# utiasSTARS/ceres-slam

Measured on AMD Instinct MI355X. Metric: gauss_newton_iters_per_sec, higher is better.
Workload: dtype f64

## Files before the change

ceres_slam_amd/csrc/ssba_api.hip:

```cpp
#include <hip/hip_runtime.h>

#include <algorithm>
#include <chrono>
#include <cmath>
#include <cstdio>
#include <cstdlib>
#include <cstring>
#include <map>
#include <condition_variable>
#include <memory>
#include <mutex>
#include <system_error>
#include <thread>
#include <string>
#include <vector>

#include "../../include/ssba.h"
#include "ssba_pool.h"
#include <dlfcn.h>
#include <rccl/rccl.h>

#include "ssba_launch.h"
#include "ssba_layout.h"
#include "ssba_wide_layout.h"
// ... 956 lines not shown
            if (f >= 0 && (f / SBP < d.chain0 || f / SBP > d.chain1)) {
                set_error("ssba_set_partition: an observation of this rank touches a pose outside its chain of super-blocks");
                return SSBA_ERR_INVALID_ARGUMENT;
            }
        }
    }
    {
        int n = part ? d.chain1 - d.chain0 + 1 : d.Nsb, lev = 0;
        const size_t c0 = part ? (size_t)d.chain0 : 0;
        d.lev[0].n = n;
        d.lev[0].D = d.xv + d.off_D + c0 * blk;
        d.lev[0].L = d.xv + d.off_L + c0 * blk;
        d.lev[0].r = d.xv + d.off_rhs + c0 * BD;
        std::vector<int> pos(n);
        for (int i = 0; i < n; ++i) pos[i] = i;
        for (;;) {
            if (d.nb) TRY(dzero(p, &d.lev[lev].B, (size_t)d.np * n * BD * NBP));
            TRY(dzero(p, &d.lev[lev].YU, (size_t)std::max(1, n / 2) * blk));
            TRY(upload_pos(pos, &d.lev[lev].pos));
            if (part ? n <= pcr_max : n == 1) break;
            d.lev[lev].pin = (part && d.pin1 && (n % 2 == 0)) ? 1 : 0;
            const int n2 = d.lev[lev].pin ? n / 2 + 1 : (n + 1) / 2;
            std::vector<int> pos2(n2);
            for (int m = 0; m < n2; ++m) pos2[m] = (d.lev[lev].pin && m == n2 - 1) ? pos[n - 1] : pos[2 * m];
            ++lev;
            if (lev >= MAX_LEVELS) return SSBA_ERR_UNSUPPORTED;
            d.lev[lev].n = n2;
            TRY(dzero(p, &d.lev[lev].D, (size_t)n2 * blk));
            TRY(dzero(p, &d.lev[lev].L, (size_t)n2 * blk));
            TRY(dzero(p, &d.lev[lev].r, (size_t)n2 * BD));
            n = n2;
            pos.swap(pos2);
        }
        d.n_levels = lev + 1;
    }
    d.pcr.level = -1;
    auto make_pcr = [&](PcrPlan &P, int level, int n, int keep, int pin0, int pin1) -> int {
        P.level = level; P.n = n; P.steps = 0; P.keep = keep; P.pin0 = pin0; P.pin1 = pin1;
        for (int s2 = 1; s2 < n; s2 <<= 1) ++P.steps;
        const size_t slots = keep ? (size_t)std::max(P.steps, 1) * n : (size_t)n;
        TRY(dzero(p, &P.Lbuf, (size_t)n * blk)); TRY(dzero(p, &P.LbufT, (size_t)n * blk));
        TRY(dzero(p, &P.YL, slots * blk)); TRY(dzero(p, &P.YU, slots * blk));
        TRY(dzero(p, &P.yr, (size_t)n * BD));
        if (pin1) TRY(dzero(p, &P.Ubuf, (size_t)n * blk));
        if (keep) {
            TRY(dzero(p, &P.Gs, slots * blk));
            const size_t np = d.nb ? (size_t)d.np : 1;
            TRY(dzero(p, &P.Bb, np * n * BD * NBP)); TRY(dzero(p, &P.yB, np * n * BD * NBP));
        }
        return SSBA_OK;
    };
    auto make_fused = [&](PcrFused &F, size_t n, bool pins) -> int {
        for (int q = 0; q < 2; ++q) {
            TRY(dzero(p, &F.Dpp[q], n * blk)); TRY(dzero(p, &F.rpp[q], n * BD));
            TRY(dzero(p, &F.GLL[q], n * blk)); TRY(dzero(p, &F.GUU[q], n * blk));
            TRY(dzero(p, &F.GUL[q], n * blk)); TRY(dzero(p, &F.GULT[q], n * blk));
            TRY(dzero(p, &F.gL[q], n * BD)); TRY(dzero(p, &F.gU[q], n * BD));
        }
        if (pins) { TRY(dzero(p, &F.Lkeep, n * blk)); TRY(dzero(p, &F.Ukeep, n * blk)); }
        F.on = 1;
        return SSBA_OK;
    };
    {
        const char *e = getenv("SSBA_NO_PCR");
        if (part) {
            TRY(make_pcr(d.pcr, d.n_levels - 1, d.lev[d.n_levels - 1].n, 0, d.pin0, d.pin1));
            if (!d.nb) TRY(make_fused(d.pcrf, (size_t)d.pcr.n, true));
        } else if ((!d.nb || d.lev[0].n <= pcr_max) && p->world_size == 1 && !dense && !(e && e[0] == '1')) {
            int k = 0;
            while (d.lev[k].n > pcr_max) ++k;
            TRY(make_pcr(d.pcr, k, d.lev[k].n, d.nb ? 1 : 0, 0, 0));
            if (!d.nb) TRY(make_fused(d.pcrf, (size_t)d.pcr.n, false));
        }
    }
    if (part) {
        const uint64_t ns = (uint64_t)d.n_sep;
        d.soff_D = 0;
        d.soff_L = d.soff_D + ns * blk;
        d.soff_rhs = d.soff_L + ns * blk;
        d.soff_gp = d.soff_rhs + ns * BD;
        d.soff_hdiag = d.soff_gp + ns * BD;
        d.soff_scal = d.soff_hdiag + ns * BD;
        d.sepv_count = d.soff_scal + NSCAL + (uint64_t)d.world;
        TRY(dzero(p, &d.sepv, d.sepv_count));
        TRY(dzero(p, &d.xsep, (size_t)ns * BD));
        d.slev[0].n = d.n_sep;
        d.slev[0].D = d.sepv + d.soff_D;
        d.slev[0].L = d.sepv + d.soff_L;
        d.slev[0].r = d.sepv + d.soff_rhs;
        std::vector<int> pos(d.n_sep);
        for (int i = 0; i < d.n_sep; ++i) pos[i] = i;
        TRY(upload_pos(pos, &d.slev[0].pos));
        TRY(make_pcr(d.spcr, 0, d.n_sep, 0, 0, 0));
        TRY(make_fused(d.spcrf, (size_t)ns, false));
    }
    std::vector<uint32_t> dn_blk_rf_start, dn_blk_rf;
    if (!pfs.empty()) {
        std::vector<uint32_t> start(P + 1, 0);
        for (auto &f : pfs) start[f.pose + 1]++;
        for (uint32_t k = 0; k < P; ++k) start[k + 1] += start[k];
        std::vector<uint32_t> cur(start.begin(), start.end() - 1);
        const size_t F = pfs.size();
        std::vector<int> type(F);
        std::vector<double> data(F * 18), S(F * 36), hub(F);
        std::vector<uint32_t> pos(F);
        for (size_t i = 0; i < F; ++i) pos[i] = cur[pfs[i].pose]++;
        for (size_t i = 0; i < F; ++i) {
            auto &f = pfs[i];
            const uint32_t q = pos[i];
            type[q] = f.type; hub[q] = f.huber;
            memcpy(&data[18 * (size_t)q], f.data, sizeof f.data);
            if (f.type >= 2 && f.data[14] >= 0.0) data[18 * (size_t)q + 14] = (double)pos[(size_t)f.data[14]];
// ... 1466 lines not shown
```

ceres_slam_amd/csrc/ssba_bcr_mfma.hip:

```cpp
#include <hip/hip_runtime.h>
#include <math.h>
#include <stdint.h>
#include <algorithm>

#include "ssba_device.h"
#include "ssba_launch.h"
#include "ssba_types.h"

namespace ssba {

typedef double mf_d4 __attribute__((ext_vector_type(4)));

static __device__ __forceinline__ mf_d4 mf(double a, double b, mf_d4 c) { return __builtin_amdgcn_mfma_f64_16x16x4f64(a, b, c, 0, 0, 0); }
static __device__ __forceinline__ double mf_readlane(double v, int lane) {
    const int lo = __builtin_amdgcn_readlane(__double2loint(v), lane);
    const int hi = __builtin_amdgcn_readlane(__double2hiint(v), lane);
    return __hiloint2double(hi, lo);
}
static __device__ __forceinline__ double mf_rcp(double a) {
    double r = __builtin_amdgcn_rcp(a);
    return fma(fma(-a, r, 1.0), r, r);
}
static __device__ __forceinline__ double mf_rsqrt(double a) {
    double r = __builtin_amdgcn_rsq(a);
    r = r * (1.5 - 0.5 * a * r * r);
    r = r * (1.5 - 0.5 * a * r * r);
    return r;
}

#ifdef SSBA_STAMPS
#define MF_STAMP(i) do { if (bx == 3 && by == 0 && (threadIdx.x & 63) == 0) d.dbg[(threadIdx.x >> 6) * 64 + (i)] = clock64(); } while (0)
#define MF_WG_STAMP(k) do { if (threadIdx.x == 0 && blockIdx.x < 500) d.dbg[4096 + 8 * (int)blockIdx.x + (k)] = wall_clock64(); } while (0)
#else
#define MF_STAMP(i) do { } while (0)
#define MF_WG_STAMP(k) do { } while (0)
#endif

static __device__ __forceinline__ void xcd_map(int id, int n, int ny, int &e, int &y) {
    const int N = n * ny, c = id & 7;
    const int q = (N + 7) >> 3, r = (N + 7) & 7;
    int idx = (id >> 3) + c * q - max(0, c - (r + 1));
    e = 0; y = 0;
#pragma unroll
    for (int k = 0; k < 8; ++k) {
        const int sk = ((n - k + 7) >> 3) * ny;
        if (idx < sk) {
            const int bq = ny == 1 ? idx : ny == 2 ? (idx >> 1) : ny == 3 ? ((idx * 0xAAAB) >> 17) : ((idx * 0x4000) >> 16);
            y = idx - bq * ny;
            e = k + 8 * bq;
            return;
        }
        idx -= sk;
    }
}
static int xcd_grid(int n, int ny) { return n * ny; }

constexpr int MF_THREADS = 256;
constexpr int NDT = 5;
constexpr int NRT = 9;

struct FactorOps {
    const double *Dg, *Lg, *Ug, *rin, *Bg;
    double *oD, *oYL, *oYU, *orr, *saveU, *oYB, *xsol;
    int f0;
    bool hasL, hasU, trL, trU;
    const double *GA, *GB, *ga, *gb;
    double sgnL, sgnU;
    double *nD, *nr, *oGLL, *oGUU, *oGUL, *oGULT, *ogL, *ogU;
    double *saveL;
    bool pinned, gLL, gUU, gUL;
};

static __device__ __forceinline__ bool factor_ops(const Dev &d, int lev, int top, int which, int bx, bool copier, bool ride, FactorOps &o) {
    o.trL = o.trU = false;
    o.saveU = nullptr;
    o.Bg = nullptr; o.oYB = nullptr; o.xsol = nullptr;
    o.GA = o.GB = o.ga = o.gb = nullptr; o.sgnL = o.sgnU = 1.0; o.nD = o.nr = nullptr;
    o.saveL = nullptr; o.pinned = false; o.gLL = o.gUU = o.gUL = false;
    if (which >= 2) {
        const PcrPlan &P = which == 3 ? d.spcr : d.pcr;
        const BcrLevel &B = which == 3 ? d.slev[0] : d.lev[d.pcr.level];
        const int blk = bx, s = 1 << lev, last = B.n - 1;
        if (P.pin0 && lev == 0 && blk == 1 && copier) {
            const double2 *s2 = reinterpret_cast<const double2 *>(B.L + (size_t)BD * BD);
            double2 *d2 = reinterpret_cast<double2 *>(P.Lbuf + (size_t)BD * BD);
            for (int e = threadIdx.x; e < BD * BD / 2; e += MF_THREADS) d2[e] = s2[e];
        }
        if ((P.pin0 && blk == 0) || (P.pin1 && blk == last)) return false;
        o.hasL = blk - s >= 0 || (P.pin0 && blk > 0);
        o.hasU = blk + s <= last || (P.pin1 && blk < last);
        o.Dg = B.D + (size_t)blk * BD * BD;
        o.rin = B.r + (size_t)blk * BD;
        if (lev == 0) {
            o.Lg = B.L + (size_t)blk * BD * BD;
            o.Ug = B.L + (size_t)(o.hasU ? blk + 1 : blk) * BD * BD;
            o.trL = o.trU = (blk & 1) == 0;
        } else {
            o.Lg = P.Lbuf + (size_t)blk * BD * BD;
            o.Ug = (P.pin1 && blk + s > last) ? P.Ubuf + (size_t)blk * BD * BD : P.LbufT + (size_t)(o.hasU ? blk + s : blk) * BD * BD;
        }
        if (P.pin1 && blk + s == last) o.saveU = P.Ubuf + (size_t)blk * BD * BD;
        const size_t so = P.keep ? (size_t)lev * B.n + blk : (size_t)blk;
        o.oD = top ? B.D + (size_t)blk * BD * BD : (P.keep ? P.Gs + so * BD * BD : nullptr);
        o.oYL = o.hasL ? P.YL + so * BD * BD : nullptr;
        o.oYU = o.hasU ? P.YU + so * BD * BD : nullptr;
        o.orr = top ? B.r + (size_t)blk * BD : P.yr + (size_t)blk * BD;
        if (ride && which == 2) { o.Bg = P.Bb + (size_t)blk * BD * NBP; o.oYB = P.yB + (size_t)blk * BD * NBP; }
        if (top && which == 2) {
            o.xsol = d.x0 + (size_t)d.chain0 * BD + (size_t)B.pos[blk] * BD;
            o.f0 = (d.chain0 + B.pos[blk]) * SBP;
        }
    } else {
        const BcrLevel &L = d.lev[lev];
        const int blk = top ? 0 : 2 * bx + 1;
        o.hasL = !top;
        o.hasU = !top && (blk + 1 < L.n);
        o.Dg = L.D + (size_t)blk * BD * BD;
        o.Lg = L.L + (size_t)blk * BD * BD;
        o.Ug = L.L + (size_t)(o.hasU ? blk + 1 : blk) * BD * BD;
        o.rin = L.r + (size_t)blk * BD;
        o.oD = L.D + (size_t)blk * BD * BD;
        o.oYL = o.hasL ? L.L + (size_t)blk * BD * BD : nullptr;
        o.oYU = top ? nullptr : L.YU + (size_t)bx * BD * BD;
        o.orr = L.r + (size_t)blk * BD;
        if (ride) { o.Bg = L.B + (size_t)blk * BD * NBP; o.oYB = L.B + (size_t)blk * BD * NBP; }
    }
    return true;
}

static __device__ __forceinline__ void fused_ops(const Dev &d, int which, int lev, int top, int bx, FactorOps &o) {
    const PcrPlan &P = which == 3 ? d.spcr : d.pcr;
    const PcrFused &F = which == 3 ? d.spcrf : d.pcrf;
    const BcrLevel &B = which == 3 ? d.slev[0] : d.lev[P.level];
    const size_t blk = (size_t)BD * BD;
    const int s = 1 << lev, h = s >> 1, last = B.n - 1, e = bx;
    const int lo = P.pin0 ? 1 : 0, hi = P.pin1 ? last - 1 : last;
    o.saveU = o.saveL = nullptr; o.Bg = nullptr; o.oYB = nullptr; o.xsol = nullptr;
    o.oYL = o.oYU = nullptr;
    o.GA = o.GB = o.ga = o.gb = nullptr;
    o.nD = o.nr = nullptr;
    o.pinned = e < lo || e > hi;
    const bool pinned_chain = P.pin0 || P.pin1;
    o.hasL = e >= 1 && (e - s >= 0 || P.pin0);
    o.hasU = e <= last - 1 && (e + s <= last || P.pin1);
    if (o.pinned) {
        o.hasU = false;
        o.hasL = e == last && e >= 1 && P.pin0 && P.pin1;
    }
    o.trL = o.trU = false;
    o.sgnL = o.sgnU = 1.0;
    o.Lg = B.L + e * blk; o.Ug = B.L + e * blk;
    if (lev == 0) {
        o.Dg = B.D + e * blk; o.rin = B.r + (size_t)e * BD;
        o.Lg = B.L + e * blk; o.Ug = B.L + (size_t)(e < last ? e + 1 : e) * blk;
        o.trL = o.trU = (e & 1) == 0;
    } else {
        const int set = (lev - 1) & 1, prev = e - h, next = e + h;
        o.Dg = lev == 1 ? B.D + e * blk : F.Dpp[(lev - 1) & 1] + e * blk;
        o.rin = lev == 1 ? B.r + (size_t)e * BD : F.rpp[(lev - 1) & 1] + (size_t)e * BD;
        if (prev >= lo) { o.GA = F.GUU[set] + prev * blk; o.ga = F.gU[set] + (size_t)prev * BD; }
        if (next <= hi) { o.GB = F.GLL[set] + next * blk; o.gb = F.gL[set] + (size_t)next * BD; }
        if (o.hasL) { if (prev >= lo) { o.Lg = F.GUL[set] + prev * blk; o.sgnL = -1.0; } else o.Lg = F.Lkeep + e * blk; }
        if (o.hasU) { if (next <= hi) { o.Ug = F.GULT[set] + next * blk; o.sgnU = -1.0; } else o.Ug = F.Ukeep + e * blk; }
        if (!top) { o.nD = F.Dpp[lev & 1] + e * blk; o.nr = F.rpp[lev & 1] + (size_t)e * BD; }
    }
    if (pinned_chain && !top) {
        if (o.hasL && e - s < lo && o.Lg != F.Lkeep + e * blk) o.saveL = F.Lkeep + e * blk;
        if (o.hasU && e + s > hi && o.Ug != F.Ukeep + e * blk) o.saveU = F.Ukeep + e * blk;
    }
    o.gLL = o.hasL && e - s >= 0 && !top;
    o.gUU = o.hasU && e + s <= last && !top;
    o.gUL = o.hasL && o.hasU && !top;
    o.oD = top ? B.D + e * blk : nullptr;
    o.orr = top ? B.r + (size_t)e * BD : nullptr;
    if (top) {
        o.xsol = which == 3 ? d.xsep + (size_t)B.pos[e] * BD : d.x0 + (size_t)d.chain0 * BD + (size_t)B.pos[e] * BD;
        o.f0 = (d.chain0 + B.pos[e]) * SBP;
        if (pinned_chain) {
            o.xsol = nullptr;
            o.oYL = o.hasL ? P.YL + e * blk : nullptr;
            o.oYU = o.hasU ? P.YU + e * blk : nullptr;
            if (o.pinned) { o.nD = B.D + e * blk; o.nr = B.r + (size_t)e * BD; }
            if (o.pinned && e == last && P.pin0 && P.pin1) o.saveL = P.Lbuf + e * blk;
        }
    }
    const int oset = lev & 1;
    o.oGLL = F.GLL[oset] + e * blk; o.oGUU = F.GUU[oset] + e * blk;
    o.oGUL = F.GUL[oset] + e * blk; o.oGULT = F.GULT[oset] + e * blk;
    o.ogL = F.gL[oset] + (size_t)e * BD; o.ogU = F.gU[oset] + (size_t)e * BD;
}

struct FactorLds {
    double P[NDT][4][64], Q[NDT][4][64];
    double A[NDT - 1][4][4][64];
    double rc[80], rs[80];
    int seqPQ;
    int seqA[4];
    int seqY[8];
    int bad;
};

#define MF_WAIT_GE(word, v)                                                                                              \
    do {                                                                                                                 \
        int it_ = 0;                                                                                                     \
        while (__builtin_amdgcn_readfirstlane(__hip_atomic_load(&(word), __ATOMIC_RELAXED, __HIP_MEMORY_SCOPE_WORKGROUP)) < (v)) { \
            if (++it_ > (1 << 20)) { S.bad = 2; break; }                                                                 \
            __builtin_amdgcn_s_sleep(1);                                                                                 \
        }                                                                                                                \
        asm volatile("" ::: "memory");                                                                                   \
        __builtin_amdgcn_sched_barrier(0);                                                                               \
    } while (0)
#define MF_POST(word, v)                                                                                                 \
    do {                                                                                                                 \
        asm volatile("" ::: "memory");                                                                                   \
        __builtin_amdgcn_sched_barrier(0);                                                                               \
        __hip_atomic_store(&(word), (v), __ATOMIC_RELAXED, __HIP_MEMORY_SCOPE_WORKGROUP);                                \
        __builtin_amdgcn_sched_barrier(0);                                                                               \
    } while (0)

#define MF_FENCE() do { asm volatile("" ::: "memory"); __builtin_amdgcn_sched_barrier(0); } while (0)

static __device__ __forceinline__ void gram_tile(int u, int &kind, int &ti, int &tj);
static __device__ __forceinline__ void gram_store(const FactorOps &o, int kind, int ti, int tj, const double (&v)[4], double *scr, int lane);
constexpr int MF_THREADS2 = 512;
template <int NRW, int MODE, int ROLE>
static __device__ __forceinline__ void factor_body(const Dev &d, FactorLds &S, double *mf_solve_lds, int lev, int top, int which, int nblocks, int ns, int rlo, int nrt, int solve) {
    constexpr bool HAS_D = ROLE != 2, HAS_R = ROLE != 1;
    State &st = *d.st;
    const StateFlags sf = state_flags_vmem(d.st);
    FactorOps o;
    int bx, by;
    xcd_map((int)blockIdx.x, nblocks, ns, bx, by);
    if (MODE) fused_ops(d, which, lev, top, bx, o);
    else if (!factor_ops(d, lev, top, which, bx, by == 0, nrt > NRT, o)) return;
    const int t = threadIdx.x, lane = t & 63, g = lane >> 4, j = lane & 15;
    const int w = __builtin_amdgcn_readfirstlane(t >> 6);
    constexpr bool rwave = HAS_R;
    const bool storeG = by == 0;
    const int rfirst = MODE == 2 ? 0 : rlo + (by * (nrt - rlo)) / ns;
    const int rcnt = MODE == 2 ? NRT : rlo + ((by + 1) * (nrt - rlo)) / ns - rfirst;
    constexpr int NRA = NRW > 0 ? NRW : 1;
    int rcol[NRA];
    bool ract[NRA];
#pragma unroll
    for (int q = 0; q < NRW; ++q) {
        const int idx = (MODE == 2 ? (w & 3) : ((w + 3) & 3)) + 4 * q;
        rcol[q] = rfirst + idx;
        ract[q] = rwave && idx < rcnt && ((rcol[q] <= 4 && o.hasL) || (rcol[q] >= 4 && rcol[q] < NRT && o.hasU) || (rcol[q] >= NRT && o.Bg));
    }
    const int dj = !HAS_D ? -1 : w == 0 ? 4 : w;
    if (t == 0) { S.bad = 0; S.seqPQ = 0; }
    if (t < 4) S.seqA[t] = 0;
    if (t < 8) { S.rc[72 + t] = 1.0; S.seqY[t] = 0; }
    if (MODE == 2) {
        for (int i = t; i < 2 * BD * 8; i += MF_THREADS2) mf_solve_lds[(i >> 3) * 80 + BD + (i & 7)] = 0.0;
    }
    __syncthreads();
    MF_STAMP(0);

    mf_d4 dt[NDT], d00, rt[NRA][NDT];
    {
        const int colD = 16 * max(dj, 0) + j;
        const int offD = g * BD + min(colD, BD - 1);
        double rv[MODE ? 1 : NDT][4];
        if (HAS_D && !MODE) {
            const double *pD = o.Dg + offD, *pr = o.rin + g;
#pragma unroll
            for (int q = 0; q < 4; ++q) d00[q] = (w == 0) ? o.Dg[(4 * q + g) * BD + j] : 0.0;
#pragma unroll
            for (int k = 0; k < NDT; ++k)
#pragma unroll
                for (int q = 0; q < 4; ++q) {
                    const bool in = k < 4 || q < 2;
                    dt[k][q] = (in && k <= dj) ? pD[(16 * k + 4 * q) * BD] : 0.0;
                    rv[k][q] = (in && w == 0) ? pr[16 * k + 4 * q] : 0.0;
                }
        }
        if (HAS_D && MODE) {
            const bool isD = colD < BD, isR = colD == BD;
            const long rstride = isD ? BD : 1, off0 = isD ? offD : g;
            const double *b0 = isD ? o.Dg : o.rin, *b1 = isD ? o.GA : o.ga, *b2 = isD ? o.GB : o.gb;
            const bool act = isD || isR;
            mf_d4 x1[NDT], x2[NDT], y1, y2;
#pragma unroll
            for (int q = 0; q < 4; ++q) {
                d00[q] = (w == 0) ? o.Dg[(4 * q + g) * BD + j] : 0.0;
                y1[q] = (w == 0 && o.GA) ? o.GA[(4 * q + g) * BD + j] : 0.0;
                y2[q] = (w == 0 && o.GB) ? o.GB[(4 * q + g) * BD + j] : 0.0;
            }
#pragma unroll
            for (int k = 0; k < NDT; ++k)
#pragma unroll
                for (int q = 0; q < 4; ++q) {
                    const bool in = (k < 4 || q < 2) && k <= dj && act;
                    const long off = off0 + (16 * k + 4 * q) * rstride;
                    dt[k][q] = in ? b0[off] : 0.0;
                    x1[k][q] = (in && b1) ? b1[off] : 0.0;
                    x2[k][q] = (in && b2) ? b2[off] : 0.0;
                }
#pragma unroll
            for (int q = 0; q < 4; ++q) d00[q] = d00[q] - y1[q] - y2[q];
#pragma unroll
            for (int k = 0; k < NDT; ++k)
#pragma unroll
                for (int q = 0; q < 4; ++q) dt[k][q] = dt[k][q] - x1[k][q] - x2[k][q];
        }
        if (!HAS_D) {
            d00 = mf_d4{0.0, 0.0, 0.0, 0.0};
#pragma unroll
            for (int k = 0; k < NDT; ++k) dt[k] = mf_d4{0.0, 0.0, 0.0, 0.0};
        }
        bool rok[NRA];
#pragma unroll
        for (int q = 0; q < NRW; ++q) {
            const int col = 16 * rcol[q] + j;
            const bool isL = col < BD, isB = rcol[q] >= NRT;
            const int cc = isL ? col : col - BD;
            const bool tr = isL ? o.trL : o.trU;
            const double *base = isL ? o.Lg : o.Ug;
            rok[q] = ract[q] && (isB || (isL ? o.hasL : o.hasU));
            if (!ract[q]) {
#pragma unroll
                for (int k = 0; k < NDT; ++k) rt[q][k] = mf_d4{0.0, 0.0, 0.0, 0.0};
            } else if (isB) {
                const double *pp = o.Bg + g * NBP + (col - 2 * BD);
#pragma unroll
                for (int k = 0; k < NDT; ++k)
#pragma unroll
                    for (int qq = 0; qq < 4; ++qq) rt[q][k][qq] = (k < 4 || qq < 2) ? pp[(16 * k + 4 * qq) * NBP] : 0.0;
            } else if (tr) {
                const double *pp = base + cc * BD + g;
#pragma unroll
                for (int k = 0; k < NDT; ++k)
#pragma unroll
                    for (int qq = 0; qq < 4; ++qq) rt[q][k][qq] = (k < 4 || qq < 2) ? pp[16 * k + 4 * qq] : 0.0;
            } else {
                const double *pp = base + g * BD + cc;
#pragma unroll
                for (int k = 0; k < NDT; ++k)
#pragma unroll
                    for (int qq = 0; qq < 4; ++qq) rt[q][k][qq] = (k < 4 || qq < 2) ? pp[(16 * k + 4 * qq) * BD] : 0.0;
            }
        }
        if (sf.dead()) return;
        if (!MODE && dj == 4) {
#pragma unroll
            for (int k = 0; k < NDT; ++k)
#pragma unroll
                for (int q = 0; q < 4; ++q) dt[k][q] = colD < BD ? dt[k][q] : colD == BD ? rv[k][q] : 0.0;
        }
        if (HAS_D && MODE && o.nD && by == 0) {
#pragma unroll
            for (int k = 0; k < NDT; ++k)
#pragma unroll
                for (int q = 0; q < 4; ++q) {
                    if (!((k < 4 || q < 2) && k <= dj)) continue;
                    if (colD < BD) {
                        o.nD[offD + (16 * k + 4 * q) * BD] = dt[k][q];
                        if (MODE == 1 && o.pinned && k < dj) o.nD[(size_t)colD * BD + 16 * k + 4 * q + g] = dt[k][q];
                    } else if (colD == BD) o.nr[g + 16 * k + 4 * q] = dt[k][q];
                }
            if (w == 0) {
#pragma unroll
                for (int q = 0; q < 4; ++q) o.nD[(4 * q + g) * BD + j] = d00[q];
            }
        }
        if (HAS_R && MODE) {
#pragma unroll
            for (int q = 0; q < NRW; ++q) {
                const double sg = (16 * rcol[q] + j < BD) ? o.sgnL : o.sgnU;
#pragma unroll
                for (int k = 0; k < NDT; ++k)
#pragma unroll
                    for (int qq = 0; qq < 4; ++qq) rt[q][k][qq] *= sg;
            }
        }
#pragma unroll
        for (int q = 0; q < NRW; ++q) {
            if (!ract[q]) continue;
            if (!rok[q]) {
#pragma unroll
                for (int k = 0; k < NDT; ++k)
#pragma unroll
                    for (int qq = 0; qq < 4; ++qq) rt[q][k][qq] = 0.0;
            }
            const int col = 16 * rcol[q] + j;
            const bool saver = MODE != 2 || by == 0;
            if (o.saveU && rok[q] && col >= BD && rcol[q] < NRT && saver) {
                double *ps = o.saveU + g * BD + col - BD;
#pragma unroll
                for (int k = 0; k < NDT; ++k)
#pragma unroll
                    for (int qq = 0; qq < 4; ++qq)
                        if (k < 4 || qq < 2) ps[(16 * k + 4 * qq) * BD] = rt[q][k][qq];
            }
            if (MODE && o.saveL && rok[q] && col < BD && saver) {
                double *ps = o.saveL + g * BD + col;
#pragma unroll
                for (int k = 0; k < NDT; ++k)
#pragma unroll
                    for (int qq = 0; qq < 4; ++qq)
                        if (k < 4 || qq < 2) ps[(16 * k + 4 * qq) * BD] = rt[q][k][qq];
            }
        }
        if (MODE && o.pinned) return;
    }

    auto mk = [](bool c) { return c ? 0xFFFFFFFFu : 0u; };
    const uint32_t mG0 = mk(g == 0), mG1 = mk(g == 1), mG2 = mk(g == 2), mG3 = mk(g == 3);
    const uint32_t mDiag = mk(j < 4 && g == j);
    const uint32_t m10 = mk(j == 1 && g == 0), m20 = mk(j == 2 && g == 0), m21 = mk(j == 2 && g == 1);
    const uint32_t m30 = mk(j == 3 && g == 0), m31 = mk(j == 3 && g == 1), m32 = mk(j == 3 && g == 2);
    const double kDiag = mDiag ? 1.0 : 0.0, k10 = m10 ? 1.0 : 0.0, k20 = m20 ? 1.0 : 0.0, k21 = m21 ? 1.0 : 0.0;
    const double k30 = m30 ? 1.0 : 0.0, k31 = m31 ? 1.0 : 0.0, k32 = m32 ? 1.0 : 0.0;
    const double kG0 = mG0 ? 1.0 : 0.0, kG1 = mG1 ? 1.0 : 0.0, kG2 = mG2 ? 1.0 : 0.0, kG3 = mG3 ? 1.0 : 0.0;
    auto sel = [](double v, uint32_t m, double acc) {
        const uint32_t lo = ((uint32_t)__double2loint(v) & m) | (uint32_t)__double2loint(acc);
        const uint32_t hi = ((uint32_t)__double2hiint(v) & m) | (uint32_t)__double2hiint(acc);
        return __hiloint2double((int)hi, (int)lo);
    };
    auto factor_tile = [&](mf_d4 &T, int k, int nsub) {
#pragma unroll
        for (int r = 0; r < 4; ++r) {
            if (r >= nsub) break;
            const int b = 4 * r;
            const double tr = T[r];
            const double s00 = mf_readlane(tr, b), s10 = mf_readlane(tr, 16 + b), s20 = mf_readlane(tr, 32 + b), s30 = mf_readlane(tr, 48 + b);
            const double s11 = mf_readlane(tr, 16 + b + 1);
            double s21 = mf_readlane(tr, 32 + b + 1), s31 = mf_readlane(tr, 48 + b + 1);
            const double s22 = mf_readlane(tr, 32 + b + 2);
            double s32 = mf_readlane(tr, 48 + b + 2);
            const double s33 = mf_readlane(tr, 48 + b + 3);
            const double x0 = __builtin_amdgcn_rcp(s00), e0 = fma(-s00, x0, 1.0);
            const double t10 = s10 * x0, t20 = s20 * x0, t30 = s30 * x0;
            const double l10 = fma(t10, e0, t10), l20 = fma(t20, e0, t20), l30 = fma(t30, e0, t30);
            const double d1 = fma(-s10, l10, s11);
            s21 = fma(-s20, l10, s21); s31 = fma(-s30, l10, s31);
            const double x1 = __builtin_amdgcn_rcp(d1), e1 = fma(-d1, x1, 1.0);
            const double t21 = s21 * x1, t31 = s31 * x1;
            const double l21 = fma(t21, e1, t21), l31 = fma(t31, e1, t31);
// ... 392 lines not shown
static __device__ __forceinline__ void stage_issue(StageRegs &R, const double *__restrict__ src, const double *__restrict__ yv) {
    const double2 *s2 = reinterpret_cast<const double2 *>(src);
#pragma unroll
    for (int q = 0; q < STAGE_NLD; ++q) {
        const int e = threadIdx.x + q * MF_THREADS;
        R.v[q] = (src && e < BD * BD / 2) ? s2[e] : make_double2(0.0, 0.0);
    }
    R.y = (threadIdx.x < BD && yv) ? yv[threadIdx.x] : 0.0;
}
static __device__ __forceinline__ void stage_write(double *dst, const StageRegs &R) {
#pragma unroll
    for (int q = 0; q < STAGE_NLD; ++q) {
        const int e = threadIdx.x + q * MF_THREADS;
        if (e >= BD * BD / 2) continue;
        const int r = (2 * e) / BD, c = 2 * e - r * BD;
        *reinterpret_cast<double2 *>(dst + r * RS + c) = R.v[q];
    }
    if (threadIdx.x < BD) {
        double *p = dst + threadIdx.x * RS + BD;
        p[0] = R.y;
#pragma unroll
        for (int c = 1; c < 8; ++c) p[c] = 0.0;
    }
}

struct TnOps { double a[BD / 4], b[BD / 4]; };
static __device__ __forceinline__ void tn_load(TnOps &O, const double *sA, const double *sB, int ti, int tj, int g, int j) {
    const double *pa = sA + g * RS + 16 * ti + j, *pb = sB + g * RS + 16 * tj + j;
#pragma unroll
    for (int s = 0; s < BD / 4; ++s) { O.a[s] = pa[4 * s * RS]; O.b[s] = pb[4 * s * RS]; }
}
static __device__ __forceinline__ mf_d4 tn_mma(const TnOps &O, mf_d4 acc) {
#pragma unroll
    for (int s = 0; s < BD / 4; ++s) acc = mf(O.a[s], O.b[s], acc);
    return acc;
}

static __device__ __forceinline__ void gram_tile(int u, int &kind, int &ti, int &tj) {
    kind = u < 15 ? 0 : u < 30 ? 1 : 2;
    if (kind == 2) {
        const int c = u - 30;
        ti = c / 5;
        tj = c - 5 * ti;
    } else {
        const int n = u - 15 * kind;
        const int a = n >= 14 ? 4 : n >= 12 ? 3 : n >= 9 ? 2 : n >= 5 ? 1 : 0;
        const int st0 = a == 4 ? 14 : a == 3 ? 12 : a == 2 ? 9 : a == 1 ? 5 : 0;
        ti = a;
        tj = min(a + (n - st0), NDT - 1);
    }
}
static __device__ __forceinline__ void gram_store(const FactorOps &o, int kind, int ti, int tj, const double (&v)[4], double *scr, int lane) {
    const int g = lane >> 4, j = lane & 15;
    const int r0 = 16 * ti + g, c0 = 16 * tj + j;
    if (kind < 2) {
        double *dst = kind == 0 ? o.oGLL : o.oGUU, *gv = kind == 0 ? o.ogL : o.ogU;
        if (c0 < BD) {
#pragma unroll
            for (int q = 0; q < 4; ++q)
                if (r0 + 4 * q < BD) dst[(r0 + 4 * q) * BD + c0] = v[q];
        } else if (c0 == BD) {
#pragma unroll
            for (int q = 0; q < 4; ++q)
                if (r0 + 4 * q < BD) gv[r0 + 4 * q] = v[q];
        }
        return;
    }
    if (c0 < BD) {
#pragma unroll
        for (int q = 0; q < 4; ++q)
            if (r0 + 4 * q < BD) o.oGUL[(r0 + 4 * q) * BD + c0] = v[q];
    }
#pragma unroll
    for (int q = 0; q < 4; ++q) scr[j * 17 + 4 * q + g] = v[q];
    MF_FENCE();
    double r[4];
#pragma unroll
    for (int q = 0; q < 4; ++q) r[q] = scr[(4 * q + g) * 17 + j];
    MF_FENCE();
    const int r1 = 16 * tj + g, c1 = 16 * ti + j;
    if (c1 < BD) {
#pragma unroll
        for (int q = 0; q < 4; ++q)
            if (r1 + 4 * q < BD) o.oGULT[(r1 + 4 * q) * BD + c1] = r[q];
    }
}

struct ReduceJob {
    const double *a0, *ya0, *a1, *ya1, *a2;
    const double *dbase, *rbase;
    double *dout, *rout;
    double *out, *outT;
    bool sym, cpl;
    const double *yb0, *yb1, *bbase;
    double *bout;
};
constexpr int BRS = 40;

#ifdef SSBA_STAMPS
#define RJ_STAMP(i) do { if (stamp_here && (threadIdx.x & 63) == 0) dbg[2048 + (threadIdx.x >> 6) * 64 + 16 * wg + (i)] = clock64(); } while (0)
#else
#define RJ_STAMP(i) do { } while (0)
#endif
static __device__ __forceinline__ void reduce_job(const ReduceJob &J, double *lds, int wg, int nwg, const StateFlags &sf, unsigned long long *dbg, bool stamp_here) {
    double *sA0 = lds, *sA1 = lds + BD * RS, *sA2 = lds + 2 * BD * RS;
    const int t = threadIdx.x, lane = t & 63, g = lane >> 4, j = lane & 15, w = t >> 6;
    const int W = 4 * wg + w, NW = 4 * nwg;
    RJ_STAMP(0);
    StageRegs R0, R1, R2;
    stage_issue(R0, (J.sym || J.cpl) ? J.a0 : nullptr, J.sym ? J.ya0 : nullptr);
    stage_issue(R1, J.sym ? J.a1 : nullptr, J.sym ? J.ya1 : nullptr);
    stage_issue(R2, J.cpl ? J.a2 : nullptr, nullptr);
    if (sf.dead()) return;
    constexpr int NSYM = 2, NCPL = 4;
    int sti[NSYM], stj[NSYM], cti[NCPL], ctj[NCPL];
    bool shave[NSYM], chave[NCPL];
    double base[NSYM][4], rb[NSYM][4];
    const int nextra = (J.sym && 15 - NW > 0) ? 15 - NW : 0;
#pragma unroll
    for (int sl = 0; sl < NSYM; ++sl) {
        const int n = W + NW * sl;
        shave[sl] = J.sym && n < 15;
        const int a = n >= 14 ? 4 : n >= 12 ? 3 : n >= 9 ? 2 : n >= 5 ? 1 : 0;
        const int st0 = a == 4 ? 14 : a == 3 ? 12 : a == 2 ? 9 : a == 1 ? 5 : 0;
        sti[sl] = a;
        stj[sl] = min(a + (n - st0), NDT - 1);
#pragma unroll
        for (int q = 0; q < 4; ++q) {
            const int rowc = min(16 * sti[sl] + 4 * q + g, BD - 1), colc = min(16 * stj[sl] + j, BD - 1);
            base[sl][q] = shave[sl] ? J.dbase[rowc * BD + colc] : 0.0;
            rb[sl][q] = shave[sl] ? J.rbase[rowc] : 0.0;
        }
    }
    {
        const int light = NW - nextra;
#pragma unroll
        for (int sl = 0; sl < NCPL; ++sl) {
            int c;
// ... 321 lines not shown
```

ceres_slam_amd/csrc/ssba_types.h:

```cpp
#pragma once
#include <stddef.h>
#include <stdint.h>
#if defined(__HIPCC__)
#define SSBA_HD __host__ __device__
#else
#define SSBA_HD
#endif

namespace ssba {

constexpr int TW = 12;
constexpr int NPAIR = TW * (TW + 1) / 2;
constexpr int SBP = 12;
constexpr int BD = 6 * SBP;
constexpr int LMG = 64;
constexpr int SLAB_DOUBLES = NPAIR * 36 + TW * 6;
constexpr int MAX_LEVELS = 18;
constexpr int MAX_SLEVELS = 1;
constexpr int MAX_SEP = 65;
constexpr int NSCAL = 16;
constexpr int NBP = 32;
constexpr int NBP_MAX = 2 * NBP;
constexpr int NBQ = 7;
constexpr int NPP = 4;
// ... 12 lines not shown
    int iteration;
    int terminated, termination_type;
    int need_linearize;
    int just_linearized;
    int last_successful;
    int accepted;
    int copy_best;
    int check_count;
    int step_failed;
    int num_successful, num_unsuccessful, num_invalid;
    int log_count;
    double radius, decrease_factor;
    double x_cost, x_norm, gmax, minimum_cost;
    double candidate_cost, model_cost_change, step_norm, relative_decrease, cost_change;
    double se_minimum, se_current, se_reference, se_candidate, se_acc_ref, se_acc_cand;
    int se_num_nonmono;
    int dl_reuse;
    double initial_cost;
    double mu, alpha, dl_step_norm, grad_norm, gn_norm, g_dot_gn, beta, gamma;
    double dl_jv2, dl_jg2, dl_jvg;
    double dl_mcc;
    int sub_one_dim, sub_pad_;
    double sub_e[2][2], sub_g[2], sub_B[3];
    double ls_alpha;
    int ls_pending, ls_active, ls_steps, ls_searches;
};
constexpr int LS_PENDING = 3;

struct IterLog {
    int capacity;
    double *cost, *cost_change, *gmax, *step_norm, *relative_decrease, *radius;
    int *successful;
};

struct BcrLevel {
    int n;
    double *D, *L, *r;
    double *YU;
    double *B;
    int pin;
    const int *pos;
};

struct PcrPlan {
    int level, n, steps;
    double *Lbuf, *LbufT, *YL, *YU, *yr;
    int keep;
    double *Gs, *Bb, *yB;
    int pin0, pin1;
    double *Ubuf;
};
constexpr int PCR_MAX_BLOCKS = 128;

struct PcrFused {
    int on;
    double *Dpp[2], *rpp[2];
    double *GLL[2], *GUU[2], *GUL[2], *GULT[2];
    double *gL[2], *gU[2];
    double *Lkeep, *Ukeep;
};

constexpr int WSP = 24;
constexpr int WBD = 6 * WSP;
constexpr int WNT = WBD / 16;
constexpr int WSLAB_TILES = WNT * (WNT + 1) / 2 + WNT;
constexpr int WSLAB_DOUBLES = WSLAB_TILES * 256;
struct WideSys {
    int n, steps, n_items, n_blk;
    double *xw;
    uint64_t off_L, off_rhs, count;
    const uint32_t *item_begin, *item_end, *item_base;
    const uint32_t *slot_obs;
    double *slab;
    const uint32_t *blk_a, *blk_b, *blk_start, *blk_contrib;
    const uint32_t *prow_start, *prow_contrib;
    double *U;
    double *YL, *YU, *yr;
};

struct Dev {
    double fu, fv, cu, cv, b;
    double S[9];
    double huber_a;
    int P, nfree, Nsb, nf_pad;
    int Lpad, n_groups, n_windows, n_slabs, n_sblk;
    int n_lm_blocks;
    uint32_t n_obs;
    double *poses, *cand_poses, *best_poses, *init_poses;
    double *pts, *cand_pts, *best_pts, *init_pts;
    const int *pose_free;
    const int *free_pose;
    const double *ou, *ov, *od;
    const uint32_t *lm_mask;
    const uint32_t *lm_win;
    const uint32_t *win_pose;
    const uint32_t *pose_obs_start;
    const uint32_t *pose_obs_ref;
    double *hll, *gl, *sl;
    double *hpp, *gp;
    double *sp;
    const uint32_t *slab_win, *slab_lm_begin, *slab_lm_end;
    double *slab;
    const uint32_t *sblk_a, *sblk_b, *sblk_start, *sblk_contrib;
    const uint32_t *sblk_rf_start, *sblk_rf;
    const uint32_t *prow_start, *prow_contrib;
    double *xv;
    uint64_t off_D, off_L, off_rhs, off_gp, off_hdiag, off_scal, xv_count;
    double *x0;
    double *vp, *vl, *dl_gn;
    double *part_dl;
    int n_levels;
// ... 95 lines not shown
```

Measured before the change: 2912.

## Store fused PCR intermediates in MFMA-tile image layout for vectorized loads

Fused PCR Gram and diagonal intermediates (Dpp, GLL, GUU, GUL, GULT, Lkeep/Ukeep) now live in a tile-major image layout that matches the MFMA fragment order. Symmetric blocks keep only the upper-triangle tiles. Loads and stores become paired double2 accesses per lane instead of strided scalar gathers with bounds checks. The separate gL/gU/rpp vector buffers are dropped, and the RHS is read from the original B.r or folded into the image columns. This should cut global memory transactions and address arithmetic in the PCR factor steps, but the changed indexing and padding carry correctness risk for pinned chains and edge tiles.

```diff
diff --git a/ceres_slam_amd/csrc/ssba_api.hip b/ceres_slam_amd/csrc/ssba_api.hip
--- a/ceres_slam_amd/csrc/ssba_api.hip
+++ b/ceres_slam_amd/csrc/ssba_api.hip
@@ -1032,12 +1032,11 @@
     };
     auto make_fused = [&](PcrFused &F, size_t n, bool pins) -> int {
         for (int q = 0; q < 2; ++q) {
-            TRY(dzero(p, &F.Dpp[q], n * blk)); TRY(dzero(p, &F.rpp[q], n * BD));
-            TRY(dzero(p, &F.GLL[q], n * blk)); TRY(dzero(p, &F.GUU[q], n * blk));
-            TRY(dzero(p, &F.GUL[q], n * blk)); TRY(dzero(p, &F.GULT[q], n * blk));
-            TRY(dzero(p, &F.gL[q], n * BD)); TRY(dzero(p, &F.gU[q], n * BD));
-        }
-        if (pins) { TRY(dzero(p, &F.Lkeep, n * blk)); TRY(dzero(p, &F.Ukeep, n * blk)); }
+            TRY(dzero(p, &F.Dpp[q], n * PCR_IMG_SYM));
+            TRY(dzero(p, &F.GLL[q], n * PCR_IMG_SYM)); TRY(dzero(p, &F.GUU[q], n * PCR_IMG_SYM));
+            TRY(dzero(p, &F.GUL[q], n * PCR_IMG_FULL)); TRY(dzero(p, &F.GULT[q], n * PCR_IMG_FULL));
+        }
+        if (pins) { TRY(dzero(p, &F.Lkeep, n * PCR_IMG_FULL)); TRY(dzero(p, &F.Ukeep, n * PCR_IMG_FULL)); }
         F.on = 1;
         return SSBA_OK;
     };
diff --git a/ceres_slam_amd/csrc/ssba_bcr_mfma.hip b/ceres_slam_amd/csrc/ssba_bcr_mfma.hip
--- a/ceres_slam_amd/csrc/ssba_bcr_mfma.hip
+++ b/ceres_slam_amd/csrc/ssba_bcr_mfma.hip
@@ -29,7 +29,10 @@
 }
 
 #ifdef SSBA_STAMPS
-#define MF_STAMP(i) do { if (bx == 3 && by == 0 && (threadIdx.x & 63) == 0) d.dbg[(threadIdx.x >> 6) * 64 + (i)] = clock64(); } while (0)
+#ifndef SSBA_STAMP_BX
+#define SSBA_STAMP_BX 3
+#endif
+#define MF_STAMP(i) do { if (bx == SSBA_STAMP_BX && by == 0 && (threadIdx.x & 63) == 0) d.dbg[(threadIdx.x >> 6) * 64 + (i)] = clock64(); } while (0)
 #define MF_WG_STAMP(k) do { if (threadIdx.x == 0 && blockIdx.x < 500) d.dbg[4096 + 8 * (int)blockIdx.x + (k)] = wall_clock64(); } while (0)
 #else
 #define MF_STAMP(i) do { } while (0)
@@ -64,9 +67,10 @@
     double *oD, *oYL, *oYU, *orr, *saveU, *oYB, *xsol;
     int f0;
     bool hasL, hasU, trL, trU;
-    const double *GA, *GB, *ga, *gb;
+    const double *GA, *GB;
     double sgnL, sgnU;
-    double *nD, *nr, *oGLL, *oGUU, *oGUL, *oGULT, *ogL, *ogU;
+    double *nD, *nr, *oGLL, *oGUU, *oGUL, *oGULT;
+    bool imgD, imgR;
     double *saveL;
     bool pinned, gLL, gUU, gUL;
 };
@@ -75,7 +79,7 @@
     o.trL = o.trU = false;
     o.saveU = nullptr;
     o.Bg = nullptr; o.oYB = nullptr; o.xsol = nullptr;
-    o.GA = o.GB = o.ga = o.gb = nullptr; o.sgnL = o.sgnU = 1.0; o.nD = o.nr = nullptr;
+    o.GA = o.GB = nullptr; o.sgnL = o.sgnU = 1.0; o.nD = o.nr = nullptr; o.imgD = o.imgR = false;
     o.saveL = nullptr; o.pinned = false; o.gLL = o.gUU = o.gUL = false;
     if (which >= 2) {
         const PcrPlan &P = which == 3 ? d.spcr : d.pcr;
@@ -132,13 +136,14 @@
     const PcrPlan &P = which == 3 ? d.spcr : d.pcr;
     const PcrFused &F = which == 3 ? d.spcrf : d.pcrf;
     const BcrLevel &B = which == 3 ? d.slev[0] : d.lev[P.level];
-    const size_t blk = (size_t)BD * BD;
+    const size_t blk = (size_t)BD * BD, isym = PCR_IMG_SYM, ifull = PCR_IMG_FULL;
     const int s = 1 << lev, h = s >> 1, last = B.n - 1, e = bx;
     const int lo = P.pin0 ? 1 : 0, hi = P.pin1 ? last - 1 : last;
     o.saveU = o.saveL = nullptr; o.Bg = nullptr; o.oYB = nullptr; o.xsol = nullptr;
     o.oYL = o.oYU = nullptr;
-    o.GA = o.GB = o.ga = o.gb = nullptr;
+    o.GA = o.GB = nullptr;
     o.nD = o.nr = nullptr;
+    o.imgD = lev >= 2; o.imgR = lev >= 1;
     o.pinned = e < lo || e > hi;
     const bool pinned_chain = P.pin0 || P.pin1;
     o.hasL = e >= 1 && (e - s >= 0 || P.pin0);
@@ -156,17 +161,18 @@
         o.trL = o.trU = (e & 1) == 0;
     } else {
         const int set = (lev - 1) & 1, prev = e - h, next = e + h;
-        o.Dg = lev == 1 ? B.D + e * blk : F.Dpp[(lev - 1) & 1] + e * blk;
-        o.rin = lev == 1 ? B.r + (size_t)e * BD : F.rpp[(lev - 1) & 1] + (size_t)e * BD;
-        if (prev >= lo) { o.GA = F.GUU[set] + prev * blk; o.ga = F.gU[set] + (size_t)prev * BD; }
-        if (next <= hi) { o.GB = F.GLL[set] + next * blk; o.gb = F.gL[set] + (size_t)next * BD; }
-        if (o.hasL) { if (prev >= lo) { o.Lg = F.GUL[set] + prev * blk; o.sgnL = -1.0; } else o.Lg = F.Lkeep + e * blk; }
-        if (o.hasU) { if (next <= hi) { o.Ug = F.GULT[set] + next * blk; o.sgnU = -1.0; } else o.Ug = F.Ukeep + e * blk; }
-        if (!top) { o.nD = F.Dpp[lev & 1] + e * blk; o.nr = F.rpp[lev & 1] + (size_t)e * BD; }
+        o.Lg = o.Ug = F.GUL[set] + e * ifull;
+        o.Dg = lev == 1 ? B.D + e * blk : F.Dpp[(lev - 1) & 1] + e * isym;
+        o.rin = B.r + (size_t)e * BD;
+        if (prev >= lo) o.GA = F.GUU[set] + prev * isym;
+        if (next <= hi) o.GB = F.GLL[set] + next * isym;
+        if (o.hasL) { if (prev >= lo) { o.Lg = F.GUL[set] + prev * ifull; o.sgnL = -1.0; } else o.Lg = F.Lkeep + e * ifull; }
+        if (o.hasU) { if (next <= hi) { o.Ug = F.GULT[set] + next * ifull; o.sgnU = -1.0; } else o.Ug = F.Ukeep + e * ifull; }
+        if (!top) o.nD = F.Dpp[lev & 1] + e * isym;
     }
     if (pinned_chain && !top) {
-        if (o.hasL && e - s < lo && o.Lg != F.Lkeep + e * blk) o.saveL = F.Lkeep + e * blk;
-        if (o.hasU && e + s > hi && o.Ug != F.Ukeep + e * blk) o.saveU = F.Ukeep + e * blk;
+        if (o.hasL && e - s < lo && o.Lg != F.Lkeep + e * ifull) o.saveL = F.Lkeep + e * ifull;
+        if (o.hasU && e + s > hi && o.Ug != F.Ukeep + e * ifull) o.saveU = F.Ukeep + e * ifull;
     }
     o.gLL = o.hasL && e - s >= 0 && !top;
     o.gUU = o.hasU && e + s <= last && !top;
@@ -185,10 +191,21 @@
         }
     }
     const int oset = lev & 1;
-    o.oGLL = F.GLL[oset] + e * blk; o.oGUU = F.GUU[oset] + e * blk;
-    o.oGUL = F.GUL[oset] + e * blk; o.oGULT = F.GULT[oset] + e * blk;
-    o.ogL = F.gL[oset] + (size_t)e * BD; o.ogU = F.gU[oset] + (size_t)e * BD;
-}
+    o.oGLL = F.GLL[oset] + e * isym; o.oGUU = F.GUU[oset] + e * isym;
+    o.oGUL = F.GUL[oset] + e * ifull; o.oGULT = F.GULT[oset] + e * ifull;
+}
+
+static __device__ __forceinline__ mf_d4 img_load(const double *base, int tile, int lane) {
+    const double2 *p = reinterpret_cast<const double2 *>(base) + tile * (PCR_IMG_TILE / 2) + lane;
+    const double2 a = p[0], b = p[64];
+    return mf_d4{a.x, a.y, b.x, b.y};
+}
+static __device__ __forceinline__ void img_store(double *base, int tile, int lane, const mf_d4 &v) {
+    double2 *p = reinterpret_cast<double2 *>(base) + tile * (PCR_IMG_TILE / 2) + lane;
+    p[0] = make_double2(v[0], v[1]);
+    p[64] = make_double2(v[2], v[3]);
+}
+static __device__ __forceinline__ int img_sym_tile(int ti, int tj) { return (ti == 4 ? 14 : ti == 3 ? 12 : ti == 2 ? 9 : ti == 1 ? 5 : 0) + tj - ti; }
 
 struct FactorLds {
     double P[NDT][4][64], Q[NDT][4][64];
@@ -257,6 +274,7 @@
     }
     __syncthreads();
     MF_STAMP(0);
+    MF_WG_STAMP(6);
 
     mf_d4 dt[NDT], d00, rt[NRA][NDT];
     {
@@ -279,25 +297,37 @@
         if (HAS_D && MODE) {
             const bool isD = colD < BD, isR = colD == BD;
             const long rstride = isD ? BD : 1, off0 = isD ? offD : g;
-            const double *b0 = isD ? o.Dg : o.rin, *b1 = isD ? o.GA : o.ga, *b2 = isD ? o.GB : o.gb;
+            const double *b0 = isD ? o.Dg : o.rin;
             const bool act = isD || isR;
-            mf_d4 x1[NDT], x2[NDT], y1, y2;
-#pragma unroll
-            for (int q = 0; q < 4; ++q) {
-                d00[q] = (w == 0) ? o.Dg[(4 * q + g) * BD + j] : 0.0;
-                y1[q] = (w == 0 && o.GA) ? o.GA[(4 * q + g) * BD + j] : 0.0;
-                y2[q] = (w == 0 && o.GB) ? o.GB[(4 * q + g) * BD + j] : 0.0;
-            }
-#pragma unroll
-            for (int k = 0; k < NDT; ++k)
-#pragma unroll
-                for (int q = 0; q < 4; ++q) {
-                    const bool in = (k < 4 || q < 2) && k <= dj && act;
-                    const long off = off0 + (16 * k + 4 * q) * rstride;
-                    dt[k][q] = in ? b0[off] : 0.0;
-                    x1[k][q] = (in && b1) ? b1[off] : 0.0;
-                    x2[k][q] = (in && b2) ? b2[off] : 0.0;
+            const mf_d4 zero4 = mf_d4{0.0, 0.0, 0.0, 0.0};
+            mf_d4 x1[NDT], x2[NDT], y1 = zero4, y2 = zero4;
+            d00 = zero4;
+            if (w == 0) {
+                if (o.imgD) d00 = img_load(o.Dg, 0, lane);
+                else {
+#pragma unroll
+                    for (int q = 0; q < 4; ++q) d00[q] = o.Dg[(4 * q + g) * BD + j];
                 }
+                if (o.GA) y1 = img_load(o.GA, 0, lane);
+                if (o.GB) y2 = img_load(o.GB, 0, lane);
+            }
+#pragma unroll
+            for (int k = 0; k < NDT; ++k) {
+                const bool have = k <= dj;
+                const int tile = img_sym_tile(k, max(dj, k));
+                dt[k] = x1[k] = x2[k] = zero4;
+                if (o.imgD) {
+                    if (have) dt[k] = img_load(o.Dg, tile, lane);
+                } else {
+#pragma unroll
+                    for (int q = 0; q < 4; ++q) {
+                        const bool in = (k < 4 || q < 2) && have && act;
+                        dt[k][q] = in ? b0[off0 + (16 * k + 4 * q) * rstride] : 0.0;
+                    }
+                }
+                if (have && o.GA) x1[k] = img_load(o.GA, tile, lane);
+                if (have && o.GB) x2[k] = img_load(o.GB, tile, lane);
+            }
 #pragma unroll
             for (int q = 0; q < 4; ++q) d00[q] = d00[q] - y1[q] - y2[q];
 #pragma unroll
@@ -328,6 +358,14 @@
                 for (int k = 0; k < NDT; ++k)
 #pragma unroll
                     for (int qq = 0; qq < 4; ++qq) rt[q][k][qq] = (k < 4 || qq < 2) ? pp[(16 * k + 4 * qq) * NBP] : 0.0;
+            } else if (MODE && o.imgR) {
+                const double *pp = base + (cc >> 4) * PCR_IMG_TILE + 2 * (16 * g + (cc & 15));
+#pragma unroll
+                for (int k = 0; k < NDT; ++k) {
+                    const double2 a = *reinterpret_cast<const double2 *>(pp + 5 * k * PCR_IMG_TILE);
+                    const double2 b = *reinterpret_cast<const double2 *>(pp + 5 * k * PCR_IMG_TILE + PCR_IMG_TILE / 2);
+                    rt[q][k] = mf_d4{a.x, a.y, b.x, b.y};
+                }
             } else if (tr) {
                 const double *pp = base + cc * BD + g;
 #pragma unroll
@@ -349,7 +387,13 @@
 #pragma unroll
                 for (int q = 0; q < 4; ++q) dt[k][q] = colD < BD ? dt[k][q] : colD == BD ? rv[k][q] : 0.0;
         }
-        if (HAS_D && MODE && o.nD && by == 0) {
+        if (HAS_D && MODE == 2 && o.nD && by == 0) {
+#pragma unroll
+            for (int k = 0; k < NDT; ++k)
+                if (k <= dj) img_store(o.nD, img_sym_tile(k, max(dj, k)), lane, dt[k]);
+            if (w == 0) img_store(o.nD, 0, lane, d00);
+        }
+        if (HAS_D && MODE == 1 && o.nD && by == 0) {
 #pragma unroll
             for (int k = 0; k < NDT; ++k)
 #pragma unroll
@@ -386,6 +430,19 @@
             }
             const int col = 16 * rcol[q] + j;
             const bool saver = MODE != 2 || by == 0;
+            if (MODE == 2) {
+                double *sv = (col >= BD ? o.saveU : o.saveL);
+                if (sv && rok[q] && rcol[q] < NRT && saver) {
+                    const int cc = col < BD ? col : col - BD;
+                    double *ps = sv + (cc >> 4) * PCR_IMG_TILE + 2 * (16 * g + (cc & 15));
+#pragma unroll
+                    for (int k = 0; k < NDT; ++k) {
+                        *reinterpret_cast<double2 *>(ps + 5 * k * PCR_IMG_TILE) = make_double2(rt[q][k][0], rt[q][k][1]);
+                        *reinterpret_cast<double2 *>(ps + 5 * k * PCR_IMG_TILE + PCR_IMG_TILE / 2) = k < 4 ? make_double2(rt[q][k][2], rt[q][k][3]) : make_double2(0.0, 0.0);
+                    }
+                }
+                continue;
+            }
             if (o.saveU && rok[q] && col >= BD && rcol[q] < NRT && saver) {
                 double *ps = o.saveU + g * BD + col - BD;
 #pragma unroll
@@ -884,25 +941,13 @@
 }
 static __device__ __forceinline__ void gram_store(const FactorOps &o, int kind, int ti, int tj, const double (&v)[4], double *scr, int lane) {
     const int g = lane >> 4, j = lane & 15;
-    const int r0 = 16 * ti + g, c0 = 16 * tj + j;
+    const bool rows = ti < 4;
     if (kind < 2) {
-        double *dst = kind == 0 ? o.oGLL : o.oGUU, *gv = kind == 0 ? o.ogL : o.ogU;
-        if (c0 < BD) {
-#pragma unroll
-            for (int q = 0; q < 4; ++q)
-                if (r0 + 4 * q < BD) dst[(r0 + 4 * q) * BD + c0] = v[q];
-        } else if (c0 == BD) {
-#pragma unroll
-            for (int q = 0; q < 4; ++q)
-                if (r0 + 4 * q < BD) gv[r0 + 4 * q] = v[q];
-        }
+        img_store(kind == 0 ? o.oGLL : o.oGUU, img_sym_tile(ti, tj), lane, mf_d4{v[0], v[1], rows ? v[2] : 0.0, rows ? v[3] : 0.0});
         return;
     }
-    if (c0 < BD) {
-#pragma unroll
-        for (int q = 0; q < 4; ++q)
-            if (r0 + 4 * q < BD) o.oGUL[(r0 + 4 * q) * BD + c0] = v[q];
-    }
+    const bool cols = tj < 4 || j < 8;
+    img_store(o.oGUL, 5 * ti + tj, lane, mf_d4{cols ? v[0] : 0.0, cols ? v[1] : 0.0, (cols && rows) ? v[2] : 0.0, (cols && rows) ? v[3] : 0.0});
 #pragma unroll
     for (int q = 0; q < 4; ++q) scr[j * 17 + 4 * q + g] = v[q];
     MF_FENCE();
@@ -910,12 +955,8 @@
 #pragma unroll
     for (int q = 0; q < 4; ++q) r[q] = scr[(4 * q + g) * 17 + j];
     MF_FENCE();
-    const int r1 = 16 * tj + g, c1 = 16 * ti + j;
-    if (c1 < BD) {
-#pragma unroll
-        for (int q = 0; q < 4; ++q)
-            if (r1 + 4 * q < BD) o.oGULT[(r1 + 4 * q) * BD + c1] = r[q];
-    }
+    const bool rowsT = tj < 4, colsT = ti < 4 || j < 8;
+    img_store(o.oGULT, 5 * tj + ti, lane, mf_d4{colsT ? r[0] : 0.0, colsT ? r[1] : 0.0, (colsT && rowsT) ? r[2] : 0.0, (colsT && rowsT) ? r[3] : 0.0});
 }
 
 struct ReduceJob {
diff --git a/ceres_slam_amd/csrc/ssba_types.h b/ceres_slam_amd/csrc/ssba_types.h
--- a/ceres_slam_amd/csrc/ssba_types.h
+++ b/ceres_slam_amd/csrc/ssba_types.h
@@ -88,11 +88,14 @@
 };
 constexpr int PCR_MAX_BLOCKS = 128;
 
+constexpr int PCR_IMG_TILE = 256;
+constexpr int PCR_IMG_SYM = 15 * PCR_IMG_TILE;
+constexpr int PCR_IMG_FULL = 25 * PCR_IMG_TILE;
 struct PcrFused {
     int on;
-    double *Dpp[2], *rpp[2];
-    double *GLL[2], *GUU[2], *GUL[2], *GULT[2];
-    double *gL[2], *gU[2];
+    double *Dpp[2];
+    double *GLL[2], *GUU[2];
+    double *GUL[2], *GULT[2];
     double *Lkeep, *Ukeep;
 };
 
```

Result: faster. 2991, median of 6 (+2.7%).
